# arun-sub/genomicsbench

Measured on AMD Instinct MI355X. Metric: bsw_large_gcups, higher is better.
Workload: dtype int32

## Files before the change

genomicsbench_amd/csrc/bsw_kernels.hip:

```cpp
#include "gbx_internal.h"
#include <atomic>
#include <cstdlib>

namespace gbx {
namespace {

constexpr int NEG = -(1 << 29);
constexpr int BIGJ = 1 << 20;

constexpr int NCLS = 21;
constexpr int CLS_LDS = NCLS - 1;
constexpr int NTB = 32;
constexpr int NBIN = NCLS * NTB;
constexpr int HDR = 1024;
constexpr int REG_SCORE_LIMIT = 1 << 20;

struct BswDev {
    int o_del, e_del, o_ins, e_ins, oe_del, oe_ins, zdrop, end_bonus, w, max_mat;
    uint32_t colword[5];
    int32_t col4[5];
    uint32_t row0[5];
    uint32_t row1[5];
    uint8_t remap[24];
    uint32_t lrow[5];
    int lane_on;
};

struct BswPairs {
    const uint8_t *ref, *qer;
    const int64_t *idr, *idq;
    const int32_t *len1, *len2, *h0;
    gbx_bsw_result *out;
    int packed = 0;
};

constexpr int WS_HDR = 4 * HDR;
struct BswWork {
    int32_t *counts, *cursors, *base, *bad, *order, *wband;
    int32_t *lbase, *lrank, *lorder, *lchunk;
};

__host__ __device__ inline int cls_of(int qlen, int bound)
{
    if (qlen > 1024 || bound >= REG_SCORE_LIMIT) return CLS_LDS;
    if (qlen > 256) return 19;
    if (qlen <= 128) return (qlen - 1) >> 3;
    return qlen <= 160 ? 16 : qlen <= 192 ? 17 : 18;
}
constexpr int LANE_QMAX = 159;
constexpr int LANE_ROWS = 2 * (LANE_QMAX + 1);
constexpr int LANE_BINS = LANE_ROWS * 256;
constexpr int LANE_SCORE_LIMIT = 8192;
constexpr int LANE_COMPACT_LIMIT = 256;
constexpr int LANE_NRANGE = 5;
constexpr int LANE_RANGE_HI[2][LANE_NRANGE] = {{47, 79, 99, 135, LANE_QMAX}, {39, 79, 103, 127, LANE_QMAX}};
__host__ __device__ inline bool lane_ok(int lane_on, int qlen, int tlen, int h0, int max_mat)
{
    return lane_on && qlen >= 1 && qlen <= LANE_QMAX && tlen >= 1 && h0 >= 0 && h0 + qlen * (max_mat > 0 ? max_mat : 0) < LANE_SCORE_LIMIT;
}
__host__ __device__ inline int lane_key(int qlen, int h0, int max_mat)
{
    const int wide = h0 + qlen * (max_mat > 0 ? max_mat : 0) < LANE_COMPACT_LIMIT ? 0 : 1;
    return ((wide * (LANE_QMAX + 1) + qlen) << 8) | (h0 < 255 ? h0 : 255);
}

__host__ __device__ inline int bin_of(int cls, int tlen)
{
    const int tb = tlen >> 4;
    return cls * NTB + (NTB - 1 - (tb < NTB - 1 ? tb : NTB - 1));
}

__device__ inline int imax3(int a, int b, int c) { return max(max(a, b), c); }

template <int CTRL, int ROWMASK = 0xf, int BANKMASK = 0xf>
__device__ inline int dpp(int old, int x)
{
    return __builtin_amdgcn_update_dpp(old, x, CTRL, ROWMASK, BANKMASK, false);
}

template <int CTRL, int ROWMASK = 0xf>
__device__ inline int dppz(int x)
{
    return __builtin_amdgcn_mov_dpp(x, CTRL, ROWMASK, 0xf, true);
}

template <int LPP>
__device__ inline int group_scan_max(int x)
{
    if (LPP == 2) return max(x, dppz<0xa0>(x));
    if (LPP <= 8) {
        x = max(x, dppz<0x90>(x));
        x = max(x, dppz<0x40>(x));
        if (LPP == 8) {
            const int tot = dppz<0xff>(x);
            x = max(x, dpp<0x114, 0xf, 0xa>(0, tot));
        }
        return x;
    }
    x = max(x, dppz<0x111>(x));
    x = max(x, dppz<0x112>(x));
    x = max(x, dppz<0x114>(x));
    x = max(x, dppz<0x118>(x));
    if (LPP >= 32) x = max(x, dpp<0x142, 0xa>(NEG, x));
    if (LPP >= 64) x = max(x, dpp<0x143, 0xc>(NEG, x));
    return x;
}

template <int LPP>
__device__ inline int group_shift_up(int x, int fill, int gl)
{
    if (LPP == 16) return dpp<0x111>(fill, x);
    if (LPP < 16) { const int y = dpp<0x111>(fill, x); return gl == 0 ? fill : y; }
    int y = dpp<0x138>(fill, x);
    return gl == 0 ? fill : y;
}

template <int LPP>
__device__ inline int group_allmax(int x)
{
    if (LPP == 2) return max(x, dppz<0xb1>(x));
    if (LPP <= 8) {
        x = max(x, dppz<0xb1>(x));
        x = max(x, dppz<0x4e>(x));
        if (LPP == 8) x = max(x, dppz<0x141>(x));
        return x;
    }
    if (LPP == 16) {
        x = max(x, dppz<0x121>(x));
        x = max(x, dppz<0x122>(x));
        x = max(x, dppz<0x124>(x));
        x = max(x, dppz<0x128>(x));
        return x;
    }
    x = max(x, dpp<0x111>(x, x));
    x = max(x, dpp<0x112>(x, x));
    x = max(x, dpp<0x114>(x, x));
    x = max(x, dpp<0x118>(x, x));
    x = max(x, dpp<0x142, 0xa>(x, x));
    x = max(x, dpp<0x143, 0xc>(x, x));
    return __builtin_amdgcn_readlane(x, 63);
}

__device__ inline int band_width(const BswDev &prm, int qlen)
{
    const int n_ins = qlen * prm.max_mat + prm.end_bonus - prm.o_ins;
    const int n_del = qlen * prm.max_mat + prm.end_bonus - prm.o_del;
    const int l_ins = n_ins >= 0 ? n_ins / prm.e_ins + 1 : 1;
    const int l_del = n_del >= 0 ? n_del / prm.e_del + 1 : 1;
    return min(prm.w, min(l_ins, l_del));
}

constexpr int CLS_THREADS = 1024;
__global__ void __launch_bounds__(CLS_THREADS) bsw_classify_kernel(BswDev prm, BswPairs P, int64_t n, BswWork W, int pass)
{
    __shared__ int lcount[NBIN];
    __shared__ int lbase[NBIN];
    const int tid = threadIdx.x;
    for (int b = tid; b < NBIN; b += CLS_THREADS) lcount[b] = 0;
    __syncthreads();
    const int64_t k = (int64_t)blockIdx.x * CLS_THREADS + tid;
    int bin = -1, slot = 0;
    if (k < n) {
        const int qlen = P.len2[k], tlen = P.len1[k], h0 = P.h0[k];
        if (qlen < 0 || tlen < 0 || qlen > GBX_BSW_MAX_QLEN || tlen > GBX_BSW_MAX_TLEN) {
            if (pass == 0) {
                gbx_bsw_result r = {-1, -1, -1, -1, -1, -1};
                P.out[k] = r;
                atomicAdd(W.bad, 1);
            }
        } else if (tlen == 0 || qlen == 0) {
            if (pass == 0) {
                gbx_bsw_result r;
                r.score = h0; r.tle = 0; r.qle = 0; r.max_off = 0;
                if (tlen == 0) { r.gtle = 0; r.gscore = -1; }
                else { int left = max(h0 - (prm.o_del + prm.e_del), 0); r.gtle = 1; r.gscore = max(-1, left); }
                P.out[k] = r;
            }
        } else if (lane_ok(prm.lane_on, qlen, tlen, h0, prm.max_mat)) {
        } else {
            const int bound = max(h0, 0) + qlen * max(prm.max_mat, 0);
            bin = bin_of(prm.remap[cls_of(qlen, bound)], tlen);
            slot = atomicAdd(&lcount[bin], 1);
        }
    }
    __syncthreads();
    if (pass == 0) {
        for (int b = tid; b < NBIN; b += CLS_THREADS)
            if (lcount[b]) atomicAdd(&W.counts[b], lcount[b]);
        return;
    }
    for (int b = tid; b < NBIN; b += CLS_THREADS)
        lbase[b] = lcount[b] ? W.base[b] + atomicAdd(&W.cursors[b], lcount[b]) : 0;
    __syncthreads();
    if (bin >= 0) {
        W.order[lbase[bin] + slot] = (int)k;
        W.wband[lbase[bin] + slot] = band_width(prm, P.len2[k]);
    }
}

__global__ void __launch_bounds__(HDR) bsw_scan_kernel(BswWork W)
{
    __shared__ int tmp[HDR];
    const int tid = threadIdx.x;
    const int v = tid < NBIN ? W.counts[tid] : 0;
    tmp[tid] = v;
    __syncthreads();
    for (int d = 1; d < HDR; d <<= 1) {
        const int add = tid >= d ? tmp[tid - d] : 0;
        __syncthreads();
        tmp[tid] += add;
        __syncthreads();
    }
    if (tid <= NBIN) W.base[tid] = tmp[tid] - v;
}

constexpr int rows_min_waves(int cpl) { return cpl >= 17 ? 3 : cpl >= 12 ? 4 : cpl >= 9 ? 5 : cpl >= 7 ? 6 : cpl >= 5 ? 7 : 1; }

template <int LPP, int CPL, bool SYM>
__global__ void __launch_bounds__(256, rows_min_waves(CPL)) bsw_rows_kernel(BswDev prm, BswPairs P, BswWork W, int cls)
{
    constexpr int KB = 10;
    constexpr int GROUPS_PER_BLOCK = 256 / LPP;
    constexpr int NQ = (CPL + 3) / 4;
    static_assert(LPP * CPL <= (1 << KB), "column index must fit the key");
    static_assert(CPL <= 32, "in-lane column index uses 5 bits");

    __shared__ uint2 s_row[8];
    const int tid = threadIdx.x;
    if (tid < 8) s_row[tid] = make_uint2(prm.row0[min(tid, 4)], prm.row1[min(tid, 4)]);
    __syncthreads();

    const int gl = tid & (LPP - 1);
    const int j0 = gl * CPL;
    const int ngroups = gridDim.x * GROUPS_PER_BLOCK;
    int next = blockIdx.x * GROUPS_PER_BLOCK + tid / LPP;

    const bool direct = cls < 0;
    const int first = direct ? 0 : W.base[cls * NTB];
    const int cnt = direct ? -cls : W.base[(cls + 1) * NTB] - first;
    const int32_t *order = W.order + first;
    const int32_t *wband = W.wband + first;

    const int e_ins = prm.e_ins, e_del = prm.e_del, oe_ins = prm.oe_ins, oe_del = prm.oe_del;
    const int lane_tilt = gl * (CPL * e_ins);

    int Hs[CPL + 1], Ev[CPL];
    uint32_t Qp[NQ];
#pragma unroll
    for (int c = 0; c < CPL; ++c) { Hs[c] = 0; Ev[c] = 0; }
#pragma unroll
    for (int c = 0; c < NQ; ++c) Qp[c] = 0;

    int qlen = 1, tlen = 1, w = 0, beg = 0, end = 0, i = 0, pair = 0, lq = 0;
    int best = 0, best_i = -1, best_j = -1, g_i = -1, g_score = -1, off = 0;
    int leftv = 0;
    const uint8_t *tptr = P.ref;
    uint2 rcur = s_row[0];
    int tnext = 0;
    bool active = false, done = false;

    for (;;) {
        if (done) {
            if (gl == lq) {
                gbx_bsw_result r;
                r.score = best; r.tle = best_i + 1; r.gtle = g_i + 1; r.qle = best_j + 1;
                r.gscore = g_score; r.max_off = off;
                P.out[pair] = r;
            }
            done = false; active = false;
            tptr = P.ref; tlen = 1; i = 0;
        }
        if (!active && next < cnt) {
            pair = direct ? next : order[next];
            w = direct ? band_width(prm, P.len2[pair]) : wband[next];
            next += ngroups;
            qlen = P.len2[pair]; tlen = P.len1[pair];
            const int h0 = P.h0[pair];
            const uint8_t *q = P.qer + P.idq[pair];
            tptr = P.ref + P.idr[pair];
#pragma unroll
            for (int c = 0; c < NQ; ++c) Qp[c] = 0;
#pragma unroll
            for (int c = 0; c < CPL; ++c) {
                const int j = j0 + c;
                int qc = j < qlen ? q[j] : 0;
                qc = min(qc, 4);
                Qp[c >> 2] |= (uint32_t)qc << ((c & 3) * 8);
                Hs[c] = j == 0 ? h0 : max(h0 - oe_ins - (j - 1) * e_ins, 0);
                Ev[c] = 0;
            }
            lq = (qlen - 1) / CPL;
            leftv = h0 - prm.o_del - e_del;
            best = h0; best_i = -1; best_j = -1; g_i = -1; g_score = -1; off = 0;
            beg = 0; end = qlen; i = 0;
            rcur = s_row[min((int)tptr[0], 4)];
            tnext = tptr[min(1, tlen - 1)];
            active = true;
        }
        if (!__any(active)) break;

        const int b = max(beg, i - w);
        const int e = min(min(end, i + w + 1), qlen);
        const int left0 = b == 0 ? max(leftv, 0) : 0;
        leftv -= e_del;
        const int lo = b - j0, hi = e - j0;
// ... 354 lines not shown
            __builtin_memcpy(&v, b, 8);
            if (o & 1) v = (v >> 4) | ((uint64_t)b[8] << 60);
            auto spread = [](unsigned h) -> unsigned { return (h & 0xfu) | ((h & 0xf0u) << 4) | ((h & 0xf00u) << 8) | ((h & 0xf000u) << 12); };
            const unsigned lo = (unsigned)v, hi = (unsigned)(v >> 32);
            r.x = spread(lo & 0xffffu); r.y = spread(lo >> 16); r.z = spread(hi & 0xffffu); r.w = spread(hi >> 16);
            return r;
        };
        auto tbase = [&](int i) -> int {
            if (!PACKED) return t[i];
            const int64_t o = to + i;
            return (t[o >> 1] >> ((int)(o & 1) * 4)) & 15;
        };
        {
            uint4 wq = qpiece(0);
            int hrun = h0 - oe_ins + e_ins;
            for (int j0 = 0; j0 <= qlen; j0 += 16) {
                const uint4 cur = wq;
                if (j0 + 16 <= qlen) wq = qpiece(j0 + 16);
                const uint32_t ww[4] = {cur.x, cur.y, cur.z, cur.w};
#pragma unroll
                for (int c = 0; c < 16; c += 2) {
                    const int j = j0 + c;
                    if (j <= qlen) {
                        const uint32_t two = (ww[c >> 2] >> ((c & 3) * 8)) & 0xffffu;
                        const int c0 = j < qlen ? min((int)(two & 0xffu), 4) : 0, c1 = j + 1 < qlen ? min((int)(two >> 8), 4) : 0;
                        const int hv0 = j == 0 ? h0 : max(hrun, 0), hv1 = max(hrun - e_ins, 0);
                        hrun -= 2 * e_ins;
                        if (COMPACT) {
                            LCELL((j >> 1) * 256 + cb) = ((uint32_t)hv0 << 8) | ((uint32_t)hv1 << 24);
                            if (CODE4) LQ8(qb + (j >> 1) * QROW) = (uint8_t)(c0 | (c1 << 4));
                            else LCELL16(qb + (j >> 1) * QROW) = (uint16_t)(c0 | (c1 << 8));
                        } else {
                            LCELL(cell_at(j)) = ((uint32_t)hv0 << 18) | (uint32_t)(c0 * 6);
                            if (j + 1 <= qlen) LCELL(cell_at(j + 1)) = ((uint32_t)hv1 << 18) | (uint32_t)(c1 * 6);
                        }
                    }
                }
            }
        }
        const int w = band_width(prm, qlen);
        int best = h0, best_i = -1, best_j = -1, g_i = -1, g_score = -1, off = 0;
        int beg = 0, end = qlen;
        uint4 mrow = LTAB(tbase(0)), mnext = LTAB(tbase(1));
        int tb2 = tbase(2);
        const uint8_t *tp = t + 3;
        int hrow = h0 - prm.o_del - e_del;
        int imw = -w, ipw = w + 1;
        for (int i = 0; i < tlen; ++i) {
            const uint32_t rw = COMPACT ? mrow.x : mrow.z, rwn = mrow.y;
            mrow = mnext;
            mnext = LTAB(tb2);
            if (PACKED) tb2 = tbase(i + 3);
            else tb2 = *tp++;
            beg = max(beg, imw);
            end = min(min(end, ipw), qlen);
            ++imw; ++ipw;
#ifdef GBX_BSW_LANE_STATS
            if (have) { st_cells += (unsigned)max(end - beg, 0); st_rows += 1; atomicMax(&st_rowmax[i & 2047], max(end - beg, 0) + 1); }
#endif
            int left = beg == 0 ? max(hrow, 0) : 0;
            hrow -= e_del;
            int f = 0;
            uint32_t key = 0;
            int vzero = 0;
            asm volatile("" : "+v"(vzero));
            uint32_t sb0 = 0, sb1 = 0, se0 = 0, se1 = 0;
            const int sp0 = beg >> 1, sq = max((end >> 1) - 1, 0);
            if (COMPACT) {
                auto step = [&](int diag, int e, uint32_t qc, int at) -> uint32_t {
                    const int sc = (int)(int8_t)__builtin_amdgcn_perm(rwn, rw, qc);
                    const int m = diag ? diag + sc : 0;
                    const int h = imax3(m, e, f);
                    key = max(key, ((uint32_t)h << 18) | (uint32_t)at);
                    const int td = m - oe_del;
                    const int en = imax3(e - e_del, td, 0);
                    f = imax3(f - e_ins, SYM ? td : m - oe_ins, 0);
                    const uint32_t cell = ((uint32_t)left << 8) | (uint32_t)en;
                    left = h;
                    return cell;
                };
                const bool odd_first = (beg & 1) && beg < end;
                int j = odd_first ? beg - 1 : beg;
                int pa = (j >> 1) * 256 + cb, qa = qb + (j >> 1) * QROW;
                uint32_t w0 = LCELL(pa), q0 = LQREAD(qa), w1 = LCELL(pa + 256), q1 = LQREAD(qa + QROW);
                w0 &= odd_first ? 0xffff0000u : 0xffffffffu;
                for (; j + 7 < end; j += 8, pa += 1024, qa += 4 * QROW) {
                    const uint32_t x0 = LCELL(pa + 512), y0 = LQREAD(qa + 2 * QROW), x1 = LCELL(pa + 768), y1 = LQREAD(qa + 3 * QROW);
                    uint32_t kt;
                    LCELL(pa) = lane_pair_step<SYM>(w0, QSEL(q0), rw, rwn, f, left, (uint32_t)vzero, kt, rel0, rel1, vzero, oe_del, oe_ins, e_del, e_ins);
                    LCELL(pa + 256) = lane_pair_step<SYM>(w1, QSEL(q1), rw, rwn, f, left, kt, kt, rel2, rel3, vzero, oe_del, oe_ins, e_del, e_ins);
                    w0 = LCELL(pa + 1024); q0 = LQREAD(qa + 4 * QROW); w1 = LCELL(pa + 1280); q1 = LQREAD(qa + 5 * QROW);
                    LCELL(pa + 512) = lane_pair_step<SYM>(x0, QSEL(y0), rw, rwn, f, left, kt, kt, rel4, rel5, vzero, oe_del, oe_ins, e_del, e_ins);
                    LCELL(pa + 768) = lane_pair_step<SYM>(x1, QSEL(y1), rw, rwn, f, left, kt, kt, rel6, rel7, vzero, oe_del, oe_ins, e_del, e_ins);
                    key = max(key, kt + (uint32_t)pa);
                }
                if (j + 3 < end) {
                    const uint32_t x0 = LCELL(pa + 512), y0 = LQREAD(qa + 2 * QROW);
                    LCELL(pa) = lane_pair_step<SYM>(w0, QSEL(q0), rw, rwn, f, left, key, key, pa, pa + 2, vzero, oe_del, oe_ins, e_del, e_ins);
                    LCELL(pa + 256) = lane_pair_step<SYM>(w1, QSEL(q1), rw, rwn, f, left, key, key, pa + 256, pa + 258, vzero, oe_del, oe_ins, e_del, e_ins);
                    w0 = x0; q0 = y0;
                    w1 = LCELL(pa + 768); q1 = LQREAD(qa + 3 * QROW);
                    j += 4; pa += 512; qa += 2 * QROW;
                }
                if (j + 1 < end) {
                    LCELL(pa) = lane_pair_step<SYM>(w0, QSEL(q0), rw, rwn, f, left, key, key, pa, pa + 2, vzero, oe_del, oe_ins, e_del, e_ins);
                    w0 = w1; q0 = q1;
                    j += 2; pa += 256; qa += QROW;
                }
                if (j < end) {
                    LCELL16(pa) = (uint16_t)step((int)((w0 >> 8) & 0xffu), (int)(w0 & 0xffu), QLOW(q0), pa);
                }
                LCELL16(cell_at(end)) = (uint16_t)(left << 8);
                sb0 = LCELL(sp0 * 256 + cb); sb1 = LCELL(sp0 * 256 + 256 + cb);
                se0 = LCELL(sq * 256 + cb); se1 = LCELL(sq * 256 + 256 + cb);
            } else {
                uint32_t left18 = (uint32_t)left << 18;
                int ab = cell_at(beg);
                const int abend = cell_at(end);
                uint32_t cw = LCELL(ab);
#pragma unroll 2
                for (; ab < abend; ab += 256) {
                    const uint32_t nw = LCELL(ab + 256);
                    const int diag = (int)(cw >> 18), e = (int)((cw >> 5) & 0x1fffu);
                    const uint32_t qo = cw & 31u;
                    const int sc = __builtin_amdgcn_sbfe((int)rw, qo, 6u);
                    const int m = diag ? diag + sc : 0;
                    const int h = imax3(m, e, f);
                    const uint32_t h18 = (uint32_t)h << 18;
                    key = max(key, h18 | (uint32_t)ab);
                    const int td = m - oe_del;
                    const int en = imax3(e - e_del, td, 0);
                    f = imax3(f - e_ins, SYM ? td : m - oe_ins, 0);
                    LCELL(ab) = left18 | ((uint32_t)en << 5) | qo;
                    left18 = h18;
                    cw = nw;
                }
                left = (int)(left18 >> 18);
                LCELL(abend) = left18 | (LCELL(abend) & 31u);
            }
            const int jfin = beg < end ? end : beg;
            if (jfin == qlen) {
                if (!(g_score > left)) g_i = i;
                g_score = max(g_score, left);
            }
            const int row_best = (int)(key >> 18);
            const int karg = (int)(key & 0x3ffffu) - cb;
            const int row_arg = COMPACT ? ((karg >> 8) << 1) | ((karg >> 1) & 1) : karg >> 8;
            if (row_best == 0) break;
            if (row_best > best) {
                best = row_best; best_i = i; best_j = row_arg;
                off = max(off, abs(row_arg - i));
            } else if (prm.zdrop > 0) {
                const int di = i - best_i, dj = row_arg - best_j;
                if (di > dj) { if (best - row_best - (di - dj) * e_del > prm.zdrop) break; }
                else if (best - row_best - (dj - di) * e_ins > prm.zdrop) break;
            }
            int j = beg;
            if (COMPACT) {
                int k = (sb1 >> 16) ? 3 : 4;
                k = (sb1 & 0xffffu) ? 2 : k;
                k = (sb0 >> 16) ? 1 : k;
                k = (sb0 & 0xffffu) && !(beg & 1) ? 0 : k;
                j = 2 * sp0 + k;
                if (k == 4) while (j < end && LCELL16(cell_at(j)) == 0) ++j;
                j = min(j, end);
                const int nbeg = beg < end ? j : beg;
                const int khi = end - 2 * sq;
                k = (se0 & 0xffffu) ? 0 : -1;
                k = (se0 >> 16) && khi >= 1 ? 1 : k;
                k = (se1 & 0xffffu) && khi >= 2 ? 2 : k;
                k = (se1 >> 16) && khi >= 3 ? 3 : k;
                j = 2 * sq + k;
                if (k < 0 && 2 * sq > nbeg) while (j >= nbeg && LCELL16(cell_at(j)) == 0) --j;
                j = max(j, nbeg - 1);
                j = nbeg > end ? end : j;
                beg = nbeg;
            } else {
                while (j < end && LCELL(cell_at(j)) < 32u) ++j;
                beg = j;
                j = end;
                while (j >= beg && LCELL(cell_at(j)) < 32u) --j;
            }
            end = min(j + 2, qlen);
        }
        gbx_bsw_result r;
        r.score = best; r.tle = best_i + 1; r.gtle = g_i + 1; r.qle = best_j + 1; r.gscore = g_score; r.max_off = off;
        if (have) P.out[pair] = r;
#ifdef GBX_BSW_LANE_STATS
        __builtin_amdgcn_s_waitcnt(0);
        for (int k = threadIdx.x; k < 2048; k += 64) { const int m = st_rowmax[k]; if (m) { st_wcells += 64ull * (unsigned)(m - 1); st_wrows += 64; } st_rowmax[k] = 0; }
#endif
    }
#ifdef GBX_BSW_LANE_STATS
    atomicAdd(&g_bsw_lane_stats[slot][0], st_cells); atomicAdd(&g_bsw_lane_stats[slot][1], st_wcells);
    atomicAdd(&g_bsw_lane_stats[slot][2], st_rows); atomicAdd(&g_bsw_lane_stats[slot][3], st_wrows);
#endif
#undef LCELL
#undef LCELL16
#undef LQ8
#undef LTAB
}


#define GBX_REG_STEP_HEAD(SEL0, SEL1)                                                                                                   \
    "v_cmp_ne_u32_sdwa vcc, %[w], %[zero] src0_sel:BYTE_1 src1_sel:DWORD\n"                                                            \
    "v_subrev_u32 %[fd], %[eins], %[f]\n"                                                                                               \
    "v_add_u32_sdwa %[ta], sext(%[sa]), %[w] dst_sel:DWORD dst_unused:UNUSED_PAD src0_sel:" SEL0 " src1_sel:BYTE_1\n"                  \
    "v_cndmask_b32 %[ma], 0, %[ta], vcc\n"                                                                                              \
    "v_cmp_ne_u32_sdwa vcc, %[w], %[zero] src0_sel:BYTE_3 src1_sel:DWORD\n"                                                            \
    "v_max_i32_sdwa %[x], %[ma], %[w] dst_sel:DWORD dst_unused:UNUSED_PAD src0_sel:DWORD src1_sel:BYTE_0\n"                            \
    "v_add_u32_sdwa %[tb], sext(%[sa]), %[w] dst_sel:DWORD dst_unused:UNUSED_PAD src0_sel:" SEL1 " src1_sel:BYTE_3\n"                  \
    "v_max_i32 %[ha], %[x], %[f]\n"
#define GBX_REG_STEP_SYM(SEL0, SEL1)                                                                                                    \
    GBX_REG_STEP_HEAD(SEL0, SEL1)                                                                                                       \
    "v_subrev_u32 %[td], %[oed], %[ma]\n"                                                                                               \
    "v_cndmask_b32 %[mb], 0, %[tb], vcc\n"                                                                                              \
    "v_sub_u32_sdwa %[ed], %[w], %[edel] dst_sel:DWORD dst_unused:UNUSED_PAD src0_sel:BYTE_0 src1_sel:DWORD\n"                         \
    "v_max3_i32 %[f], %[fd], %[td], 0\n"                                                                                                \
    "v_max3_i32 %[ena], %[ed], %[td], 0\n"                                                                                              \
    "v_max_i32_sdwa %[x], %[mb], %[w] dst_sel:DWORD dst_unused:UNUSED_PAD src0_sel:DWORD src1_sel:BYTE_2\n"                            \
    "v_lshl_or_b32 %[ka], %[ha], 18, %[pa]\n"                                                                                           \
    "v_max_i32 %[hb], %[x], %[f]\n"                                                                                                     \
    "v_subrev_u32 %[td], %[oed], %[mb]\n"                                                                                               \
    "v_subrev_u32 %[fd], %[eins], %[f]\n"                                                                                               \
    "v_sub_u32_sdwa %[ed], %[w], %[edel] dst_sel:DWORD dst_unused:UNUSED_PAD src0_sel:BYTE_2 src1_sel:DWORD\n"                         \
    "v_max3_i32 %[f], %[fd], %[td], 0\n"                                                                                                \
    "v_max3_i32 %[enb], %[ed], %[td], 0\n"                                                                                              \
    "v_lshl_or_b32 %[kb], %[hb], 18, %[pa1]\n"                                                                                          \
    "v_lshl_or_b32 %[u], %[left], 8, %[ena]\n"                                                                                          \
    "v_lshl_or_b32 %[v], %[ha], 8, %[enb]\n"                                                                                            \
    "v_max3_u32 %[key], %[kin], %[ka], %[kb]\n"                                                                                         \
    "v_lshl_or_b32 %[wn], %[v], 16, %[u]\n"
#define GBX_REG_STEP_ASYM(SEL0, SEL1)                                                                                                   \
    GBX_REG_STEP_HEAD(SEL0, SEL1)                                                                                                       \
    "v_subrev_u32 %[td], %[oed], %[ma]\n"                                                                                               \
    "v_subrev_u32 %[ti], %[oei], %[ma]\n"                                                                                               \
    "v_cndmask_b32 %[mb], 0, %[tb], vcc\n"                                                                                              \
    "v_sub_u32_sdwa %[ed], %[w], %[edel] dst_sel:DWORD dst_unused:UNUSED_PAD src0_sel:BYTE_0 src1_sel:DWORD\n"                         \
    "v_max3_i32 %[f], %[fd], %[ti], 0\n"                                                                                                \
    "v_max3_i32 %[ena], %[ed], %[td], 0\n"                                                                                              \
    "v_max_i32_sdwa %[x], %[mb], %[w] dst_sel:DWORD dst_unused:UNUSED_PAD src0_sel:DWORD src1_sel:BYTE_2\n"                            \
    "v_lshl_or_b32 %[ka], %[ha], 18, %[pa]\n"                                                                                           \
    "v_max_i32 %[hb], %[x], %[f]\n"                                                                                                     \
    "v_subrev_u32 %[td], %[oed], %[mb]\n"                                                                                               \
    "v_subrev_u32 %[ti], %[oei], %[mb]\n"                                                                                               \
    "v_subrev_u32 %[fd], %[eins], %[f]\n"                                                                                               \
    "v_sub_u32_sdwa %[ed], %[w], %[edel] dst_sel:DWORD dst_unused:UNUSED_PAD src0_sel:BYTE_2 src1_sel:DWORD\n"                         \
    "v_max3_i32 %[f], %[fd], %[ti], 0\n"                                                                                                \
    "v_max3_i32 %[enb], %[ed], %[td], 0\n"                                                                                              \
    "v_lshl_or_b32 %[kb], %[hb], 18, %[pa1]\n"                                                                                          \
    "v_lshl_or_b32 %[u], %[left], 8, %[ena]\n"                                                                                          \
    "v_lshl_or_b32 %[v], %[ha], 8, %[enb]\n"                                                                                            \
    "v_max3_u32 %[key], %[kin], %[ka], %[kb]\n"                                                                                         \
    "v_lshl_or_b32 %[wn], %[v], 16, %[u]\n"
template <bool SYM, bool HI, int PA>
__device__ __forceinline__ uint32_t reg_pair_step(uint32_t w, uint32_t sa, int &f, int &left, uint32_t &key, int zero, int oe_del, int oe_ins,
                                                  int e_del, int e_ins)
{
    uint32_t wn, kout;
    int hb, ta, tb, ma, mb, x, ha, td, ti, ed, ena, enb, fd, ka, kb, u, v;
#define GBX_REG_STEP_OPS                                                                                                                \
    : [ta] "=&v"(ta), [tb] "=&v"(tb), [ma] "=&v"(ma), [mb] "=&v"(mb), [x] "=&v"(x), [ha] "=&v"(ha), [hb] "=&v"(hb), [td] "=&v"(td),   \
      [ti] "=&v"(ti), [ed] "=&v"(ed), [ena] "=&v"(ena), [enb] "=&v"(enb), [fd] "=&v"(fd), [ka] "=&v"(ka), [kb] "=&v"(kb), [u] "=&v"(u), \
      [v] "=&v"(v), [wn] "=&v"(wn), [f] "+v"(f), [key] "=v"(kout)                                                                       \
    : [w] "v"(w), [sa] "v"(sa), [left] "v"(left), [kin] "v"(key), [pa] "i"(PA), [pa1] "i"(PA + 1), [zero] "v"(zero), [oed] "s"(oe_del), \
      [oei] "s"(oe_ins), [edel] "s"(e_del), [eins] "s"(e_ins)                                                                           \
    : "vcc"
    if (SYM && !HI) asm volatile(GBX_REG_STEP_SYM("BYTE_0", "BYTE_1") GBX_REG_STEP_OPS);
    if (SYM && HI) asm volatile(GBX_REG_STEP_SYM("BYTE_2", "BYTE_3") GBX_REG_STEP_OPS);
    if (!SYM && !HI) asm volatile(GBX_REG_STEP_ASYM("BYTE_0", "BYTE_1") GBX_REG_STEP_OPS);
    if (!SYM && HI) asm volatile(GBX_REG_STEP_ASYM("BYTE_2", "BYTE_3") GBX_REG_STEP_OPS);
#undef GBX_REG_STEP_OPS
    (void)ti;
    left = hb;
    key = kout;
    return wn;
}
#undef GBX_REG_STEP_SYM
#undef GBX_REG_STEP_ASYM
#undef GBX_REG_STEP_HEAD

template <bool AND>
__device__ inline uint32_t wave_bits(uint32_t x)
{
    auto op = [](uint32_t a, uint32_t b) { return AND ? a & b : a | b; };
    int y = (int)x;
    y = (int)op(y, dpp<0x111>(y, y));
    y = (int)op(y, dpp<0x112>(y, y));
    y = (int)op(y, dpp<0x114>(y, y));
    y = (int)op(y, dpp<0x118>(y, y));
    y = (int)op(y, dpp<0x142, 0xa>(y, y));
    y = (int)op(y, dpp<0x143, 0xc>(y, y));
    return (uint32_t)__builtin_amdgcn_readlane(y, 63);
}
__device__ inline uint32_t bits_from(int lo)
{
    return lo <= 0 ? ~0u : lo >= 32 ? 0u : ~0u << lo;
}
__device__ inline uint32_t bit_span(int lo, int hi)
{
    return lo > hi ? 0u : (hi >= 31 ? ~0u : (2u << hi) - 1u) & ~((1u << lo) - 1u);
}

template <bool SYM, bool HI, int PA>
__device__ __forceinline__ void reg_pair_masked(uint32_t &cell, uint32_t sa, int beg, int end, int &f, int &left, uint32_t &key,
                                                int zero, int oe_del, int oe_ins, int e_del, int e_ins)
{
    constexpr int c0 = PA;
    if (c0 + 1 < end && c0 + 1 >= beg) {
        const uint32_t win = c0 < beg ? cell & 0xffff0000u : cell;
        cell = reg_pair_step<SYM, HI, PA>(win, sa, f, left, key, zero, oe_del, oe_ins, e_del, e_ins);
    } else if (c0 + 1 == end) {
        if (c0 >= beg) {
            const int sc = (int)(int8_t)(sa >> (HI ? 16 : 0));
            const int diag = (int)((cell >> 8) & 0xffu), e = (int)(cell & 0xffu);
            const int m = diag ? diag + sc : 0;
            const int h = imax3(m, e, f);
            key = max(key, ((uint32_t)h << 18) | (uint32_t)PA);
            const int en = imax3(e - e_del, m - oe_del, 0);
            cell = ((uint32_t)h << 24) | ((uint32_t)left << 8) | (uint32_t)en;
            left = h;
        } else {
            cell = (cell & 0xffffu) | ((uint32_t)left << 24);
        }
    } else if (c0 == end) {
        cell = (cell & 0xffff0000u) | ((uint32_t)left << 8);
    }
}

template <bool SYM, int QHI>
__global__ void __launch_bounds__(64, 3) bsw_lane_reg_kernel(BswDev prm, BswPairs P, BswWork W, int rlo, int rhi, int slot)
{
    constexpr int NCP = QHI / 2 + 1;
    constexpr int NB = (NCP + 3) / 4;
    constexpr int NQ = (NCP + 1) / 2;
    constexpr int NW = (2 * NCP + 31) / 32;
    static_assert(NB <= 31, "block masks are 32-bit");
    constexpr int OUT = 1 << 12;
    __shared__ uint2 s_tab[5];
    const int lane = threadIdx.x;
    if (lane < 5) s_tab[lane] = make_uint2(prm.row0[lane], prm.row1[lane]);
    __syncthreads();
    const int first = W.lbase[rlo << 8], count = W.lbase[(rhi + 1) << 8] - first;
    const int nchunks = (count + 63) >> 6;
    const int32_t *order = W.lorder + first;
    const int e_ins = prm.e_ins, e_del = prm.e_del, oe_ins = prm.oe_ins, oe_del = prm.oe_del;
    for (;;) {
        int c = 0;
        if (lane == 0) c = atomicAdd(&W.lchunk[slot], 1);
        c = __builtin_amdgcn_readfirstlane(c);
        if (c >= nchunks) break;
        const int hi_ = count - (c << 6), idx = hi_ - 64 + lane;
        const bool have = idx >= 0;
        const int pair = order[have ? idx : 0];
        const int qlen = P.len2[pair], tlen = P.len1[pair], h0 = P.h0[pair];
        const uint8_t *q = P.qer + P.idq[pair];
        const uint8_t *t = P.ref + P.idr[pair];

        uint32_t qs[NQ];
#pragma unroll
        for (int k = 0; k < (4 * NQ + 15) / 16; ++k) {
            uint4 v = make_uint4(0u, 0u, 0u, 0u);
            if (16 * k <= qlen) __builtin_memcpy(&v, q + 16 * k, 16);
            const uint32_t vv[4] = {v.x, v.y, v.z, v.w};
#pragma unroll
            for (int m = 0; m < 4 && 4 * k + m < NQ; ++m) {
                const uint32_t x = vv[m];
                const uint32_t ge5 = ((((x | 0x80808080u) - 0x05050505u) | x) & 0x80808080u) >> 7;
                const uint32_t msk = ge5 * 0xffu;
                qs[4 * k + m] = (x & ~msk) | (0x04040404u & msk);
            }
        }
        uint32_t cell[NCP];
        {
            int hr = h0 - oe_ins, rem = qlen;
#pragma unroll
            for (int p = 0; p < NCP; ++p) {
                const int hv0 = p == 0 ? h0 : max(hr + e_ins, 0), hv1 = max(hr, 0);
                cell[p] = (rem >= 0 ? (uint32_t)hv0 << 8 : 0u) | (rem >= 1 ? (uint32_t)hv1 << 24 : 0u);
                hr -= 2 * e_ins;
                rem -= 2;
            }
        }
        const int w = band_width(prm, qlen);
        int best = h0, best_i = -1, best_j = -1, g_i = -1, g_score = -1, off = 0;
        int beg = 0, end = qlen;
        bool running = true;
        uint2 mrow = s_tab[min((int)t[0], 4)], mnext = s_tab[min((int)t[1], 4)];
        int tb2 = t[2];
        const uint8_t *tp = t + 3;
        int hrow = h0 - prm.o_del - e_del;
        int imw = -w, ipw = w + 1;
        for (int i = 0;; ++i) {
            if (!__any(running)) break;
            const uint32_t rw = mrow.x, rwn = mrow.y;
            mrow = mnext;
            mnext = s_tab[min(tb2, 4)];
            tb2 = running ? (int)*tp : 0;
            tp += running ? 1 : 0;
            beg = max(beg, imw);
            end = min(min(end, ipw), qlen);
            ++imw; ++ipw;
            int left = beg == 0 ? max(hrow, 0) : 0;
            hrow -= e_del;
            const int bb = running ? beg : OUT, ee = running ? end : OUT;
            const int sp0 = bb >> 1, sq = max((ee >> 1) - 1, 0);
            const uint32_t touch = running ? bit_span(bb >> 3, min(ee >> 3, NB - 1)) : 0u;
            const uint32_t whole = running ? bit_span((bb + 7) >> 3, min((ee >> 3) - 1, NB - 1)) : ~0u;
            auto blk = [](int pp) { return pp < 4 * NB ? 1u << (pp >> 2) : 0u; };
            const uint32_t probe = running ? blk(sp0) | blk(sp0 + 1) | blk(sq) | blk(sq + 1) : 0u;
            const uint32_t touch_w = wave_bits<false>(touch), whole_w = wave_bits<true>(whole), probe_w = wave_bits<false>(probe);
            int vzero = 0;
            asm volatile("" : "+v"(vzero));
            int f = 0;
            uint32_t key = 0;
#pragma unroll
            for (int b = 0; b < NB; ++b) {
                if (!((touch_w >> b) & 1u)) continue;
                const uint32_t sa0 = __builtin_amdgcn_perm(rwn, rw, qs[2 * b]);
                const uint32_t sa1 = 2 * b + 1 < NQ ? __builtin_amdgcn_perm(rwn, rw, qs[2 * b + 1]) : 0u;
                uint32_t kt = (uint32_t)vzero;
                if ((whole_w >> b) & 1u) {
                    cell[4 * b] = reg_pair_step<SYM, false, 0>(cell[4 * b], sa0, f, left, kt, vzero, oe_del, oe_ins, e_del, e_ins);
                    if (4 * b + 1 < NCP) cell[4 * b + 1] = reg_pair_step<SYM, true, 2>(cell[4 * b + 1], sa0, f, left, kt, vzero, oe_del, oe_ins, e_del, e_ins);
                    if (4 * b + 2 < NCP) cell[4 * b + 2] = reg_pair_step<SYM, false, 4>(cell[4 * b + 2], sa1, f, left, kt, vzero, oe_del, oe_ins, e_del, e_ins);
                    if (4 * b + 3 < NCP) cell[4 * b + 3] = reg_pair_step<SYM, true, 6>(cell[4 * b + 3], sa1, f, left, kt, vzero, oe_del, oe_ins, e_del, e_ins);
                } else {
                    int lb = bb - 8 * b, le = ee - 8 * b;
                    asm volatile("" : "+v"(lb), "+v"(le));
                    reg_pair_masked<SYM, false, 0>(cell[4 * b], sa0, lb, le, f, left, kt, vzero, oe_del, oe_ins, e_del, e_ins);
                    if (4 * b + 1 < NCP) reg_pair_masked<SYM, true, 2>(cell[4 * b + 1], sa0, lb, le, f, left, kt, vzero, oe_del, oe_ins, e_del, e_ins);
                    if (4 * b + 2 < NCP) reg_pair_masked<SYM, false, 4>(cell[4 * b + 2], sa1, lb, le, f, left, kt, vzero, oe_del, oe_ins, e_del, e_ins);
                    if (4 * b + 3 < NCP) reg_pair_masked<SYM, true, 6>(cell[4 * b + 3], sa1, lb, le, f, left, kt, vzero, oe_del, oe_ins, e_del, e_ins);
                }
                key = max(key, kt + (uint32_t)(8 * b));
            }
            uint32_t sb0 = 0, sb1 = 0, se0 = 0, se1 = 0;
#pragma unroll
            for (int b = 0; b < NB; ++b) {
                if (!((probe_w >> b) & 1u)) continue;
                int db = sp0 - 4 * b, de = sq - 4 * b;
                asm volatile("" : "+v"(db), "+v"(de));
#pragma unroll
                for (int m = 0; m < 4 && 4 * b + m < NCP; ++m) {
                    const uint32_t cv = cell[4 * b + m];
                    sb0 = db == m ? cv : sb0;
                    sb1 = db == m - 1 ? cv : sb1;
                    se0 = de == m ? cv : se0;
                    se1 = de == m - 1 ? cv : se1;
                }
            }
            if (running) {
                const int jfin = beg < end ? end : beg;
                if (jfin == qlen) {
                    if (!(g_score > left)) g_i = i;
                    g_score = max(g_score, left);
                }
                const int row_best = (int)(key >> 18), row_arg = (int)(key & 0x3ffffu);
                bool stop = row_best == 0;
                if (!stop) {
                    if (row_best > best) {
                        best = row_best; best_i = i; best_j = row_arg;
                        off = max(off, abs(row_arg - i));
                    } else if (prm.zdrop > 0) {
                        const int di = i - best_i, dj = row_arg - best_j;
                        stop = di > dj ? best - row_best - (di - dj) * e_del > prm.zdrop : best - row_best - (dj - di) * e_ins > prm.zdrop;
                    }
                }
                if (!stop) {
                    int k = (sb1 >> 16) ? 3 : 4;
                    k = (sb1 & 0xffffu) ? 2 : k;
                    k = (sb0 >> 16) ? 1 : k;
                    k = (sb0 & 0xffffu) && !(beg & 1) ? 0 : k;
                    int j = 2 * sp0 + k;
                    const int khi = end - 2 * sq;
                    int ke = (se0 & 0xffffu) ? 0 : -1;
                    ke = (se0 >> 16) && khi >= 1 ? 1 : ke;
                    ke = (se1 & 0xffffu) && khi >= 2 ? 2 : ke;
                    ke = (se1 >> 16) && khi >= 3 ? 3 : ke;
                    uint32_t nz[NW];
                    if (k == 4 || ke < 0) {
#pragma unroll
                        for (int u = 0; u < NW; ++u) nz[u] = 0u;
#pragma unroll
                        for (int p = 0; p < NCP; ++p) {
                            const uint32_t two = ((cell[p] & 0xffffu) ? 1u : 0u) | ((cell[p] >> 16) ? 2u : 0u);
                            nz[p >> 4] |= two << ((2 * p) & 31);
                        }
                    }
                    if (k == 4) {
                        int jn = end;
#pragma unroll
                        for (int u = NW - 1; u >= 0; --u) {
                            const uint32_t m = nz[u] & bits_from(j - 32 * u) & ~bits_from(end - 32 * u);
                            jn = m ? 32 * u + __builtin_ctz(m) : jn;
                        }
                        j = jn;
                    }
                    j = min(j, end);
                    const int nbeg = beg < end ? j : beg;
                    j = 2 * sq + ke;
                    if (ke < 0 && 2 * sq > nbeg) {
                        int jl = nbeg - 1;
#pragma unroll
                        for (int u = 0; u < NW; ++u) {
                            const uint32_t m = nz[u] & bits_from(nbeg - 32 * u) & ~bits_from(j + 1 - 32 * u);
                            jl = m ? 32 * u + 31 - __builtin_clz(m) : jl;
                        }
                        j = jl;
                    }
                    j = max(j, nbeg - 1);
                    j = nbeg > end ? end : j;
                    beg = nbeg;
                    end = min(j + 2, qlen);
                }
                running = !stop && i + 1 < tlen;
            }
        }
        gbx_bsw_result r;
        r.score = best; r.tle = best_i + 1; r.gtle = g_i + 1; r.qle = best_j + 1; r.gscore = g_score; r.max_off = off;
        if (have) P.out[pair] = r;
    }
}

struct RowShape { int lpp, cpl; };
typedef void (*RowsFn)(BswDev, BswPairs, BswWork, int);
struct RowKernel { int lpp, cpl; RowsFn fn[2]; std::atomic<int> bpc[2]; const char *name; };
#define GBX_ROW_KERNEL(L, C) { L, C, { bsw_rows_kernel<L, C, false>, bsw_rows_kernel<L, C, true> }, { 0, 0 }, "bsw_rows_" #L "x" #C }
RowKernel row_kernels[] = {
    GBX_ROW_KERNEL(2, 4),  GBX_ROW_KERNEL(2, 8),  GBX_ROW_KERNEL(2, 12), GBX_ROW_KERNEL(2, 16), GBX_ROW_KERNEL(2, 20), GBX_ROW_KERNEL(2, 24),
    GBX_ROW_KERNEL(4, 14), GBX_ROW_KERNEL(4, 16), GBX_ROW_KERNEL(4, 18), GBX_ROW_KERNEL(4, 20), GBX_ROW_KERNEL(4, 22), GBX_ROW_KERNEL(4, 24),
    GBX_ROW_KERNEL(8, 13), GBX_ROW_KERNEL(8, 14), GBX_ROW_KERNEL(8, 15), GBX_ROW_KERNEL(8, 16),
    GBX_ROW_KERNEL(16, 10), GBX_ROW_KERNEL(16, 12), GBX_ROW_KERNEL(16, 16), GBX_ROW_KERNEL(64, 16),
    GBX_ROW_KERNEL(4, 8), GBX_ROW_KERNEL(4, 12), GBX_ROW_KERNEL(8, 10), GBX_ROW_KERNEL(8, 12), GBX_ROW_KERNEL(16, 8),
    GBX_ROW_KERNEL(64, 3), GBX_ROW_KERNEL(64, 4),
};
#undef GBX_ROW_KERNEL
constexpr int class_qmax[NCLS - 1] = {8, 16, 24, 32, 40, 48, 56, 64, 72, 80, 88, 96, 104, 112, 120, 128, 160, 192, 256, 1024};

constexpr uint8_t CLASS_REMAP[3][NCLS] = {
    {0, 1, 2, 3, 4, 5, 6, 7, 8, 9, 10, 11, 12, 13, 14, 15, 16, 17, 18, 19, 20},
    {3, 3, 3, 3, 7, 7, 7, 7, 11, 11, 11, 11, 15, 15, 15, 15, 18, 18, 18, 19, 20},
    {15, 15, 15, 15, 15, 15, 15, 15, 15, 15, 15, 15, 15, 15, 15, 15, 18, 18, 18, 19, 20},
};
int class_mode_for(int64_t n)
{
    const char *e = getenv("GBX_BSW_CLASSMODE");
    if (e && *e >= '0' && *e <= '2') return *e - '0';
    return n < 32768 ? 2 : n < 250000 ? 1 : 0;
}

RowKernel *find_row_kernel(int lpp, int cpl)
{
    for (RowKernel &k : row_kernels)
        if (k.lpp == lpp && k.cpl == cpl) return &k;
    return nullptr;
}

const RowShape *class_shapes()
{
    static RowShape shapes[NCLS - 1] = {{2, 4},  {2, 8},  {2, 12}, {2, 16}, {2, 20}, {2, 24}, {4, 14}, {4, 16}, {4, 18}, {4, 20},
                                        {4, 22}, {4, 24}, {8, 13}, {8, 14}, {8, 15}, {8, 16}, {16, 10}, {16, 12}, {16, 16}, {64, 16}};
    static bool parsed = false;
    if (!parsed) {
        parsed = true;
        const char *e = getenv("GBX_BSW_SHAPES");
        for (int c = 0; e && *e && c < NCLS - 1; ++c) {
            int l = 0, k = 0, used = 0;
            if (sscanf(e, "%dx%d%n", &l, &k, &used) != 2) break;
            if (find_row_kernel(l, k) && l * k >= class_qmax[c]) shapes[c] = {l, k};
            e += used;
            if (*e == ',') ++e;
        }
    }
    return shapes;
}

int make_dev_params(const gbx_bsw_params *p, BswDev *d)
{
    if (p->e_del < 1 || p->e_ins < 1 || p->o_del < 0 || p->o_ins < 0 || p->e_del > 4096 || p->e_ins > 4096 ||
        p->o_del > (1 << 16) || p->o_ins > (1 << 16) || p->w < 0) {
        set_error("bsw: gap penalties must satisfy 0<=o<=65536, 1<=e<=4096, w>=0");
        return GBX_ERR_ARG;
    }
    d->o_del = p->o_del; d->e_del = p->e_del; d->o_ins = p->o_ins; d->e_ins = p->e_ins;
    d->oe_del = p->o_del + p->e_del; d->oe_ins = p->o_ins + p->e_ins;
    d->zdrop = p->zdrop; d->end_bonus = p->end_bonus; d->w = p->w;
    int mx = 0;
    for (int k = 0; k < 25; ++k) mx = p->mat[k] > mx ? p->mat[k] : mx;
    d->max_mat = mx;
    for (int q = 0; q < 5; ++q) {
        uint32_t wv = 0;
        for (int t = 0; t < 4; ++t) wv |= (uint32_t)(uint8_t)p->mat[t * 5 + q] << (8 * t);
        d->colword[q] = wv;
        d->col4[q] = p->mat[4 * 5 + q];
    }
    for (int t = 0; t < 5; ++t) {
        uint32_t wv = 0;
        for (int q = 0; q < 4; ++q) wv |= (uint32_t)(uint8_t)p->mat[t * 5 + q] << (8 * q);
        d->row0[t] = wv;
        d->row1[t] = (uint32_t)(uint8_t)p->mat[t * 5 + 4];
    }
    d->lane_on = 0;
    bool fits6 = true;
    for (int k = 0; k < 25; ++k) fits6 = fits6 && p->mat[k] >= -32 && p->mat[k] <= 31;
    for (int t = 0; t < 5; ++t) {
        uint32_t wv = 0;
        for (int q = 0; q < 5; ++q) wv |= ((uint32_t)p->mat[t * 5 + q] & 63u) << (6 * q);
        d->lrow[t] = wv;
    }
    if (fits6 && p->o_del + p->e_del < LANE_SCORE_LIMIT && p->o_ins + p->e_ins < LANE_SCORE_LIMIT) d->lane_on = -1;
    return GBX_OK;
}

}

constexpr int64_t WS_LANE = (int64_t)(LANE_BINS + 64) + 64;
size_t bsw_workspace_bytes(int64_t n)
{
    return (size_t)(WS_HDR + 4 * (n > 0 ? n : 0) + WS_LANE) * sizeof(int32_t);
}

constexpr int UNPACK_ROUNDS = 4;
__global__ void __launch_bounds__(256) bsw_unpack4_kernel(const uint8_t *__restrict__ packed, uint8_t *__restrict__ out, int64_t lo, int64_t hi)
{
    const int64_t base = lo + (int64_t)blockIdx.x * (256 * 16 * UNPACK_ROUNDS) + threadIdx.x * 16;
    const bool aligned = (((uintptr_t)(packed + (base >> 1)) & 7) == 0) && (((uintptr_t)(out + base) & 15) == 0);
    if (aligned && base + (int64_t)(UNPACK_ROUNDS - 1) * 4096 + 16 <= hi) {
        uint2 v[UNPACK_ROUNDS];
#pragma unroll
        for (int r = 0; r < UNPACK_ROUNDS; ++r) v[r] = *(const uint2 *)(packed + ((base + r * 4096) >> 1));
        auto spread = [](unsigned h) -> unsigned { return (h & 0xfu) | ((h & 0xf0u) << 4) | ((h & 0xf00u) << 8) | ((h & 0xf000u) << 12); };
#pragma unroll
        for (int r = 0; r < UNPACK_ROUNDS; ++r) {
            uint4 q;
            q.x = spread(v[r].x & 0xffffu); q.y = spread(v[r].x >> 16); q.z = spread(v[r].y & 0xffffu); q.w = spread(v[r].y >> 16);
            *(uint4 *)(out + base + r * 4096) = q;
        }
        return;
    }
    for (int r = 0; r < UNPACK_ROUNDS; ++r) {
        const int64_t o = base + r * 4096;
        if (o >= hi) return;
        if (aligned && o + 16 <= hi) {
            const uint2 v = *(const uint2 *)(packed + (o >> 1));
            auto spread = [](unsigned h) -> unsigned { return (h & 0xfu) | ((h & 0xf0u) << 4) | ((h & 0xf00u) << 8) | ((h & 0xf000u) << 12); };
            uint4 q;
            q.x = spread(v.x & 0xffffu); q.y = spread(v.x >> 16); q.z = spread(v.y & 0xffffu); q.w = spread(v.y >> 16);
            *(uint4 *)(out + o) = q;
        } else {
            for (int64_t k = o; k < o + 16 && k < hi; ++k) out[k] = (uint8_t)((packed[k >> 1] >> ((k & 1) * 4)) & 0xf);
        }
    }
}

int bsw_unpack4(const uint8_t *d_packed, uint8_t *d_out, int64_t lo, int64_t hi, hipStream_t s)
{
    if (hi <= lo) return GBX_OK;
    const int64_t per_block = 256 * 16 * UNPACK_ROUNDS;
    Stage st("bsw_unpack4", s);
    hipLaunchKernelGGL(bsw_unpack4_kernel, dim3((unsigned)((hi - lo + per_block - 1) / per_block)), dim3(256), 0, s, d_packed, d_out, lo, hi);
    GBX_HIP(hipGetLastError());
    return GBX_OK;
}

int bsw_launch_direct(const gbx_bsw_params *p, int64_t n, int max_qlen,
                      const uint8_t *d_ref, const uint8_t *d_qer, const int64_t *d_idr, const int64_t *d_idq,
                      const int32_t *d_len1, const int32_t *d_len2, const int32_t *d_h0, gbx_bsw_result *d_out, hipStream_t s)
{
    if (n <= 0) return GBX_OK;
    BswDev dev;
    int rc = make_dev_params(p, &dev);
    if (rc) return rc;
    for (int c = 0; c < NCLS; ++c) dev.remap[c] = (uint8_t)c;
    BswPairs P = {d_ref, d_qer, d_idr, d_idq, d_len1, d_len2, d_h0, d_out};
    BswWork W = {nullptr, nullptr, nullptr, nullptr, nullptr, nullptr, nullptr, nullptr, nullptr, nullptr};
    dev.lane_on = 0;
    if (max_qlen > 256) { set_error("bsw: direct launch needs queries of at most 256"); return GBX_ERR_ARG; }
    const int cols = max_qlen + 1;
    int lpp = 16, cpl = cols <= 128 ? 8 : cols <= 160 ? 10 : cols <= 192 ? 12 : 16;
    if (n < 4096) { lpp = 64; cpl = cols <= 192 ? 3 : 4; }
    if (const char *e = getenv("GBX_BSW_DIRECT_SHAPE")) {
        int l = 0, c = 0;
        if (sscanf(e, "%dx%d", &l, &c) == 2 && l * c > max_qlen && find_row_kernel(l, c)) { lpp = l; cpl = c; }
    }
    RowKernel *k = find_row_kernel(lpp, cpl);
    if (!k) { set_error("bsw: no %dx%d row kernel", lpp, cpl); return GBX_ERR_UNSUPPORTED; }
    const bool sym = dev.oe_ins == dev.oe_del;
    const int gpb = 256 / lpp;
    const int blocks = (int)((n + gpb - 1) / gpb);
    Stage st(k->name, s);
    hipLaunchKernelGGL(k->fn[sym], dim3(blocks), dim3(256), 0, s, dev, P, W, -(int)n);
    GBX_HIP(hipGetLastError());
    return GBX_OK;
}

static std::atomic<long long> g_lane_reg_launches{0};

static bool lane_wanted(int64_t n)
{
    const char *lane_env = getenv("GBX_BSW_LANE");
    const int64_t lane_min = getenv("GBX_BSW_LANE_MIN") ? atoll(getenv("GBX_BSW_LANE_MIN")) : 262144;
    return lane_env ? atoi(lane_env) != 0 : n >= lane_min;
}

int bsw_lane_rule(const gbx_bsw_params *p, int64_t n, BswLaneRule *r)
{
    BswDev dev;
    const int rc = make_dev_params(p, &dev);
    if (rc) return rc;
    r->on = dev.lane_on && lane_wanted(n) ? 1 : 0;
    r->max_mat = dev.max_mat > 0 ? dev.max_mat : 0;
    r->qmax = LANE_QMAX;
    r->limit = LANE_SCORE_LIMIT;
    r->compact_limit = LANE_COMPACT_LIMIT;
    static_assert(LANE_NRANGE == 5, "BswLaneRule::range_hi / BswChunkPrep::class_pairs");
    for (int f = 0; f < 2; ++f) for (int k = 0; k < LANE_NRANGE; ++k) r->range_hi[f][k] = LANE_RANGE_HI[f][k];
    return GBX_OK;
}

int bsw_launch(const gbx_bsw_params *p, int64_t n,
               const uint8_t *d_ref, const uint8_t *d_qer,
               const int64_t *d_idr, const int64_t *d_idq,
               const int32_t *d_len1, const int32_t *d_len2, const int32_t *d_h0,
               gbx_bsw_result *d_out, void *d_work, size_t work_bytes, hipStream_t s, hipEvent_t *join_events,
               const BswChunkPrep *prep)
{
    if (n == 0) return GBX_OK;
    if (n > 0x7fffffffLL - 1024) { set_error("bsw: more than 2^31 pairs in one call"); return GBX_ERR_UNSUPPORTED; }
    if (work_bytes < bsw_workspace_bytes(n)) { set_error("bsw: workspace too small"); return GBX_ERR_ARG; }
    BswDev dev;
    int rc = make_dev_params(p, &dev);
    if (rc) return rc;
    const int mode = class_mode_for(n);
    for (int c = 0; c < NCLS; ++c) dev.remap[c] = CLASS_REMAP[mode][c];
    BswPairs P = {d_ref, d_qer, d_idr, d_idq, d_len1, d_len2, d_h0, d_out};
    int32_t *wi = (int32_t *)d_work;
    int32_t *wl = wi + WS_HDR + 4 * n;
    BswWork W = {wi, wi + HDR, wi + 2 * HDR, wi + 3 * HDR, wi + WS_HDR, wi + WS_HDR + n, wl, wi + WS_HDR + 3 * n, wi + WS_HDR + 2 * n,
                 wl + LANE_BINS + 64};
    dev.lane_on = dev.lane_on && lane_wanted(n) ? 1 : 0;
    static const bool serial = getenv("GBX_BSW_SERIAL") != nullptr;
    SideStreams *ss = nullptr;
    std::unique_lock<std::mutex> side_lock;
    if (!serial) {
        if ((rc = side_streams(&ss))) return rc;
        side_lock = std::unique_lock<std::mutex>(ss->mu);
    }
    static const bool prep_off = getenv("GBX_BSW_PREP") && atoi(getenv("GBX_BSW_PREP")) == 0;
    const bool ahead = prep && prep->uploaded && join_events && !serial && !prep_off;
    hipStream_t s_cls = ahead ? ss->pre[0] : s;
    const bool no_rows = dev.lane_on && prep && prep->rows_pairs == 0 && !(getenv("GBX_BSW_SKIP_ROWS") && atoi(getenv("GBX_BSW_SKIP_ROWS")) == 0);
    const bool packed_lanes = no_rows && prep->ref_packed && !(getenv("GBX_BSW_PACKED_LANES") && atoi(getenv("GBX_BSW_PACKED_LANES")) == 0);
    const int phase = prep ? prep->phase : 0;
    if (phase && !(ahead && packed_lanes && prep->ev_pre && prep->ev_aux)) {
// ... 193 lines not shown
```

Baseline: 2532.

## Process banded DP in half-blocks with LDS-table edge masks instead of per-cell branches

Changes the register-resident banded Smith-Waterman row update from 4-pair blocks with a per-pair masked path to 2-pair half-blocks. Band edges are handled by blending full step results under bit masks read from a small LDS table, so edge cases no longer need branchy scalar code. The wave-uniform mask ballots are packed so fewer cross-lane reductions run per row. The final 'left' value is recovered from the probed end cell rather than tracked through the masked path. This removes divergent edge handling and trims wasted work at block granularity, at the cost of extra LDS reads and blend operations at the edges.

```diff
diff --git a/genomicsbench_amd/csrc/bsw_kernels.hip b/genomicsbench_amd/csrc/bsw_kernels.hip
--- a/genomicsbench_amd/csrc/bsw_kernels.hip
+++ b/genomicsbench_amd/csrc/bsw_kernels.hip
@@ -1,6 +1,8 @@
 #include "gbx_internal.h"
 #include <atomic>
 #include <cstdlib>
+#include <type_traits>
+#include <utility>
 
 namespace gbx {
 namespace {
@@ -961,30 +963,33 @@
     return lo > hi ? 0u : (hi >= 31 ? ~0u : (2u << hi) - 1u) & ~((1u << lo) - 1u);
 }
 
-template <bool SYM, bool HI, int PA>
-__device__ __forceinline__ void reg_pair_masked(uint32_t &cell, uint32_t sa, int beg, int end, int &f, int &left, uint32_t &key,
-                                                int zero, int oe_del, int oe_ins, int e_del, int e_ins)
-{
-    constexpr int c0 = PA;
-    if (c0 + 1 < end && c0 + 1 >= beg) {
-        const uint32_t win = c0 < beg ? cell & 0xffff0000u : cell;
-        cell = reg_pair_step<SYM, HI, PA>(win, sa, f, left, key, zero, oe_del, oe_ins, e_del, e_ins);
-    } else if (c0 + 1 == end) {
-        if (c0 >= beg) {
-            const int sc = (int)(int8_t)(sa >> (HI ? 16 : 0));
-            const int diag = (int)((cell >> 8) & 0xffu), e = (int)(cell & 0xffu);
-            const int m = diag ? diag + sc : 0;
-            const int h = imax3(m, e, f);
-            key = max(key, ((uint32_t)h << 18) | (uint32_t)PA);
-            const int en = imax3(e - e_del, m - oe_del, 0);
-            cell = ((uint32_t)h << 24) | ((uint32_t)left << 8) | (uint32_t)en;
-            left = h;
-        } else {
-            cell = (cell & 0xffffu) | ((uint32_t)left << 24);
-        }
-    } else if (c0 == end) {
-        cell = (cell & 0xffff0000u) | ((uint32_t)left << 8);
-    }
+template <bool SYM, int MODE, int PA, bool TWO>
+__device__ __forceinline__ void reg_half(uint32_t &c0, uint32_t &c1, uint32_t sa, uint2 tl, uint2 tr, uint2 wr, int &f, int &left, uint32_t &key,
+                                         int zero, int oe_del, int oe_ins, int e_del, int e_ins)
+{
+    auto one = [&](uint32_t &c, uint32_t ml, uint32_t mr, uint32_t mw, auto hi) {
+        constexpr bool HI = decltype(hi)::value;
+        uint32_t in = c;
+        if (MODE & 2) in &= mr;
+        if (MODE & 1) in &= ~ml;
+        const uint32_t n = reg_pair_step<SYM, HI, PA + (HI ? 2 : 0)>(in, sa, f, left, key, zero, oe_del, oe_ins, e_del, e_ins);
+        if (MODE == 0) c = n;
+        if (MODE == 1) c = (ml & c) | (~ml & n);
+        if (MODE == 2) c = (mw & n) | (~mw & c);
+        if (MODE == 3) { const uint32_t m = mw & ~ml; c = (m & n) | (~m & c); }
+    };
+    one(c0, tl.x, tr.x, wr.x, std::false_type{});
+    if (TWO) one(c1, tl.y, tr.y, wr.y, std::true_type{});
+}
+template <typename F, int... I>
+__device__ __forceinline__ void static_for_seq(F &&fn, std::integer_sequence<int, I...>)
+{
+    (fn(std::integral_constant<int, I>{}), ...);
+}
+template <int N, typename F>
+__device__ __forceinline__ void static_for(F &&fn)
+{
+    static_for_seq(fn, std::make_integer_sequence<int, N>{});
 }
 
 template <bool SYM, int QHI>
@@ -994,11 +999,15 @@
     constexpr int NB = (NCP + 3) / 4;
     constexpr int NQ = (NCP + 1) / 2;
     constexpr int NW = (2 * NCP + 31) / 32;
-    static_assert(NB <= 31, "block masks are 32-bit");
+    constexpr int NH = (NCP + 1) / 2;
+    static_assert(NH <= 25 && NB <= 13, "a half mask and half of the probed blocks share a word");
+    static_assert(NQ == NH, "a selector dword serves a half block");
     constexpr int OUT = 1 << 12;
     __shared__ uint2 s_tab[5];
     const int lane = threadIdx.x;
+    __shared__ uint2 s_half[5];
     if (lane < 5) s_tab[lane] = make_uint2(prm.row0[lane], prm.row1[lane]);
+    if (lane < 5) s_half[lane] = make_uint2(lane >= 2 ? ~0u : lane == 1 ? 0xffffu : 0u, lane >= 4 ? ~0u : lane == 3 ? 0xffffu : 0u);
     __syncthreads();
     const int first = W.lbase[rlo << 8], count = W.lbase[(rhi + 1) << 8] - first;
     const int nchunks = (count + 63) >> 6;
@@ -1060,40 +1069,48 @@
             beg = max(beg, imw);
             end = min(min(end, ipw), qlen);
             ++imw; ++ipw;
-            int left = beg == 0 ? max(hrow, 0) : 0;
+            const int left0 = beg == 0 ? max(hrow, 0) : 0;
+            int left = left0;
             hrow -= e_del;
-            const int bb = running ? beg : OUT, ee = running ? end : OUT;
+            const bool live = running && beg < end;
+            const int bb = live ? beg : OUT, ee = live ? end : OUT;
             const int sp0 = bb >> 1, sq = max((ee >> 1) - 1, 0);
-            const uint32_t touch = running ? bit_span(bb >> 3, min(ee >> 3, NB - 1)) : 0u;
-            const uint32_t whole = running ? bit_span((bb + 7) >> 3, min((ee >> 3) - 1, NB - 1)) : ~0u;
+            constexpr uint32_t HMASK = (1u << NH) - 1u;
             auto blk = [](int pp) { return pp < 4 * NB ? 1u << (pp >> 2) : 0u; };
-            const uint32_t probe = running ? blk(sp0) | blk(sp0 + 1) | blk(sq) | blk(sq + 1) : 0u;
-            const uint32_t touch_w = wave_bits<false>(touch), whole_w = wave_bits<true>(whole), probe_w = wave_bits<false>(probe);
+            const uint32_t probe = live ? blk(sp0) | blk(sp0 + 1) | blk(sq) | blk(sq + 1) : 0u;
+            const uint32_t touch = live ? bit_span(bb >> 2, min(ee >> 2, NH - 1)) : 0u;
+            const uint32_t edge_l = live ? ~bits_from((bb + 3) >> 2) & HMASK : 0u;
+            const uint32_t edge_r = live ? bits_from(ee >> 2) & HMASK : 0u;
+            const uint32_t r0 = wave_bits<false>(touch | (probe & 0x7fu) << 25), r1 = wave_bits<false>(edge_l | (probe >> 7) << 25);
+            const uint32_t touch_w = r0 & HMASK, left_w = r1 & HMASK, right_w = wave_bits<false>(edge_r);
+            const uint32_t probe_w = (r0 >> 25) | (r1 >> 25) << 7;
             int vzero = 0;
             asm volatile("" : "+v"(vzero));
             int f = 0;
-            uint32_t key = 0;
-#pragma unroll
-            for (int b = 0; b < NB; ++b) {
-                if (!((touch_w >> b) & 1u)) continue;
-                const uint32_t sa0 = __builtin_amdgcn_perm(rwn, rw, qs[2 * b]);
-                const uint32_t sa1 = 2 * b + 1 < NQ ? __builtin_amdgcn_perm(rwn, rw, qs[2 * b + 1]) : 0u;
-                uint32_t kt = (uint32_t)vzero;
-                if ((whole_w >> b) & 1u) {
-                    cell[4 * b] = reg_pair_step<SYM, false, 0>(cell[4 * b], sa0, f, left, kt, vzero, oe_del, oe_ins, e_del, e_ins);
-                    if (4 * b + 1 < NCP) cell[4 * b + 1] = reg_pair_step<SYM, true, 2>(cell[4 * b + 1], sa0, f, left, kt, vzero, oe_del, oe_ins, e_del, e_ins);
-                    if (4 * b + 2 < NCP) cell[4 * b + 2] = reg_pair_step<SYM, false, 4>(cell[4 * b + 2], sa1, f, left, kt, vzero, oe_del, oe_ins, e_del, e_ins);
-                    if (4 * b + 3 < NCP) cell[4 * b + 3] = reg_pair_step<SYM, true, 6>(cell[4 * b + 3], sa1, f, left, kt, vzero, oe_del, oe_ins, e_del, e_ins);
-                } else {
-                    int lb = bb - 8 * b, le = ee - 8 * b;
-                    asm volatile("" : "+v"(lb), "+v"(le));
-                    reg_pair_masked<SYM, false, 0>(cell[4 * b], sa0, lb, le, f, left, kt, vzero, oe_del, oe_ins, e_del, e_ins);
-                    if (4 * b + 1 < NCP) reg_pair_masked<SYM, true, 2>(cell[4 * b + 1], sa0, lb, le, f, left, kt, vzero, oe_del, oe_ins, e_del, e_ins);
-                    if (4 * b + 2 < NCP) reg_pair_masked<SYM, false, 4>(cell[4 * b + 2], sa1, lb, le, f, left, kt, vzero, oe_del, oe_ins, e_del, e_ins);
-                    if (4 * b + 3 < NCP) reg_pair_masked<SYM, true, 6>(cell[4 * b + 3], sa1, lb, le, f, left, kt, vzero, oe_del, oe_ins, e_del, e_ins);
-                }
-                key = max(key, kt + (uint32_t)(8 * b));
-            }
+            uint32_t key = (uint32_t)vzero, key64 = (uint32_t)vzero;
+            const int bb8 = bb << 3, ee8 = ee << 3;
+            static_for<NH>([&](auto hc) {
+                constexpr int h = decltype(hc)::value;
+                if (!((touch_w >> h) & 1u)) return;
+                constexpr bool two = 2 * h + 1 < NCP;
+                constexpr int pa = 4 * h < 64 ? 4 * h : 4 * h - 64;
+                uint32_t &kk = 4 * h < 64 ? key : key64;
+                uint32_t &c0 = cell[2 * h], &c1 = cell[two ? 2 * h + 1 : 2 * h];
+                const uint32_t sa = __builtin_amdgcn_perm(rwn, rw, qs[h]);
+                const bool el = (left_w >> h) & 1u, er = (right_w >> h) & 1u;
+                auto row = [&](int at8) -> uint2 {
+                    int a = at8 - 32 * h;
+                    asm volatile("" : "+v"(a));
+                    return *(const uint2 *)((const char *)s_half + min(max(a, 0), 32));
+                };
+                const uint2 none = make_uint2(0u, 0u);
+                if (!el && !er) reg_half<SYM, 0, pa, two>(c0, c1, sa, none, none, none, f, left, kk, vzero, oe_del, oe_ins, e_del, e_ins);
+                else if (!er) reg_half<SYM, 1, pa, two>(c0, c1, sa, row(bb8), none, none, f, left, kk, vzero, oe_del, oe_ins, e_del, e_ins);
+                else if (!el) reg_half<SYM, 2, pa, two>(c0, c1, sa, none, row(ee8), row(ee8 + 8), f, left, kk, vzero, oe_del, oe_ins, e_del, e_ins);
+                else reg_half<SYM, 3, pa, two>(c0, c1, sa, row(bb8), row(ee8), row(ee8 + 8), f, left, kk, vzero, oe_del, oe_ins, e_del, e_ins);
+            });
+            if (NH > 16) key = max(key, key64 + 64u);
+            key = live ? key : 0u;
             uint32_t sb0 = 0, sb1 = 0, se0 = 0, se1 = 0;
 #pragma unroll
             for (int b = 0; b < NB; ++b) {
@@ -1110,6 +1127,8 @@
                 }
             }
             if (running) {
+                const uint32_t ce = end >= 2 ? se1 : se0;
+                left = live ? (int)((end & 1 ? ce >> 24 : ce >> 8) & 0xffu) : left0;
                 const int jfin = beg < end ? end : beg;
                 if (jfin == qlen) {
                     if (!(g_score > left)) g_i = i;
```

Result: no change. 2521 (-0.5%).
